# nv-tlabs/LION

Measured on AMD Instinct MI355X. Metric: shapes/sec @1000-step DDIM, Bx2048pts, higher is better.
Workload: dtype f32 (operands of the 3x3x3 voxel convolutions and of the long 1x1 convolutions cut into fp16 hi/lo pairs on the 16-bi...

## Files before the change

lion_amd/csrc/devoxelize.hip:

```cpp
#include "common.h"

namespace {

struct Corners {
  int ix[8];
  float w[8];
};

__device__ __forceinline__ Corners corners_of(float x, float y, float z, int r, int r2) {
  Corners k;
  const float xl = floorf(x), yl = floorf(y), zl = floorf(z);
  const float xd1 = sub_rn(x, xl), yd1 = sub_rn(y, yl), zd1 = sub_rn(z, zl);
  const float xd0 = sub_rn(1.0f, xd1), yd0 = sub_rn(1.0f, yd1), zd0 = sub_rn(1.0f, zd1);
  k.w[0] = mul_rn(mul_rn(xd0, yd0), zd0);
  k.w[1] = mul_rn(mul_rn(xd0, yd0), zd1);
  k.w[2] = mul_rn(mul_rn(xd0, yd1), zd0);
  k.w[3] = mul_rn(mul_rn(xd0, yd1), zd1);
  k.w[4] = mul_rn(mul_rn(xd1, yd0), zd0);
  k.w[5] = mul_rn(mul_rn(xd1, yd0), zd1);
  k.w[6] = mul_rn(mul_rn(xd1, yd1), zd0);
  k.w[7] = mul_rn(mul_rn(xd1, yd1), zd1);
  const int xlo = (int)xl, ylo = (int)yl, zlo = (int)zl;
  const int xs = (xd1 > 0.0f) ? r2 : 0;
  const int ys = (yd1 > 0.0f) ? r : 0;
  const int zs = (zd1 > 0.0f) ? 1 : 0;
  k.ix[0] = xlo * r2 + ylo * r + zlo;
  k.ix[1] = k.ix[0] + zs;
  k.ix[2] = k.ix[0] + ys;
  k.ix[3] = k.ix[2] + zs;
  k.ix[4] = k.ix[0] + xs;
  k.ix[5] = k.ix[4] + zs;
  k.ix[6] = k.ix[4] + ys;
  k.ix[7] = k.ix[6] + zs;
  return k;
}

template <int CT, bool AFF>
__global__ __launch_bounds__(256) void devox_fwd_kernel(const float *__restrict__ coords,
                                                        const float *__restrict__ feat, int C,
                                                        int N, int r, int training,
                                                        float *__restrict__ out,
                                                        int32_t *__restrict__ inds,
                                                        float *__restrict__ wgts,
                                                        const float *__restrict__ scale,
                                                        const float *__restrict__ shift) {
  const int b = blockIdx.z, i = blockIdx.x * blockDim.x + threadIdx.x;
  if (i >= N) return;
  const int r2 = r * r, r3 = r2 * r;
  const float *co = coords + (size_t)b * 3 * N;
  Corners k = corners_of(co[i], co[i + N], co[i + 2 * N], r, r2);
  if (training && blockIdx.y == 0) {
#pragma unroll
    for (int q = 0; q < 8; ++q) {
      wgts[((size_t)b * 8 + q) * N + i] = k.w[q];
      inds[((size_t)b * 8 + q) * N + i] = k.ix[q];
    }
  }
#pragma unroll
  for (int q = 0; q < 8; ++q) k.ix[q] = min(max(k.ix[q], 0), r3 - 1);
  const int c0 = blockIdx.y * CT, c1 = min(C, c0 + CT);
  const float *f = feat + ((size_t)b * C + c0) * r3;
  float *o = out + ((size_t)b * C + c0) * N + i;
  float wsum = 0.f;
  if (AFF) {
    wsum = k.w[0];
#pragma unroll
    for (int q = 1; q < 8; ++q) wsum += k.w[q];
  }
#pragma unroll 4
  for (int c = c0; c < c1; ++c, f += r3, o += N) {
    float v[8];
#pragma unroll
    for (int q = 0; q < 8; ++q) v[q] = f[k.ix[q]];
    float acc = mul_rn(k.w[0], v[0]);
#pragma unroll
    for (int q = 1; q < 8; ++q) acc = add_rn(acc, mul_rn(k.w[q], v[q]));
    if (AFF) acc = acc * scale[(size_t)b * C + c] + shift[(size_t)b * C + c] * wsum;
    *o = acc;
  }
}


template <int LD, bool AFF, bool SPLIT>
__global__ __launch_bounds__(256) void devox_slab_kernel(
    const float *__restrict__ coords, const float *__restrict__ feat, int C, int N, int r, int PX,
    int XS, int CT, int CI, int slab_floats, int training, float *__restrict__ out,
    int32_t *__restrict__ inds, float *__restrict__ wgts, const float *__restrict__ scale,
    const float *__restrict__ shift) {
  extern __shared__ __attribute__((aligned(16))) unsigned char smem[];
  float *lds = reinterpret_cast<float *>(smem);
  constexpr int PP = 8;
  const int tid = threadIdx.x, b = blockIdx.y, c0 = blockIdx.x * CT;
  const int nch = min(CT, C - c0);
  const int r2 = r * r, r3 = r2 * r;
  const float *co = coords + (size_t)b * 3 * N;
  uint16_t *sorted = reinterpret_cast<uint16_t *>(lds + 2 * slab_floats);
  int *scnt = reinterpret_cast<int *>(sorted + ((N + 1) & ~1));
  unsigned *need = reinterpret_cast<unsigned *>(scnt + XS);

  const int ngrp = (nch + CI - 1) / CI;
  const int nit = ngrp * XS;
  auto slab_count4 = [&](int g, int xs) {
    return XS == 1 ? (min(CI, nch - g * CI) * r3) >> 2 : ((min(r, xs * PX + PX + 1) - xs * PX) * r2) >> 2;
  };
  typedef __attribute__((address_space(3))) float lds_float;
  const uint32_t lds_base = (uint32_t)(uintptr_t)(lds_float *)lds;
  const int wave = __builtin_amdgcn_readfirstlane(tid >> 6);
  auto issue = [&](int it) {
    const int g = it / XS, xs = it - g * XS;
    const float4 *src = reinterpret_cast<const float4 *>(feat + ((size_t)b * C + c0 + g * CI) * r3 + (size_t)xs * PX * r2);
    const int n4 = slab_count4(g, xs);
    const uint32_t dst0 = lds_base + (uint32_t)((it & 1) * slab_floats * 4 + wave * 1024);
    const int row0 = XS == 1 ? 0 : xs * PX * r;
#pragma unroll
    for (int j = 0; j < LD; ++j) {
      const int f = tid + j * 256;
      const float4 *gp = src + f;
      const uint32_t dst = __builtin_amdgcn_readfirstlane(dst0 + j * 4096);
      int row = (4 * f) / r;
      if (XS == 1) row %= r2;
      else row += row0;
      bool want = f < n4 && ((need[row >> 5] >> (row & 31)) & 1u);
      if (SPLIT && !want && f < n4) {
        int rowh = (4 * f + 3) / r;
        if (XS == 1) rowh %= r2;
        else rowh += row0;
        want = (need[rowh >> 5] >> (rowh & 31)) & 1u;
      }
      if (want) {
        unsigned keep;
        asm volatile("s_mov_b32 %0, m0\n\ts_mov_b32 m0, %2\n\ts_nop 0\n\tglobal_load_lds_dwordx4 %1, off\n\ts_mov_b32 m0, %0"
                     : "=&s"(keep) : "v"(gp), "s"(dst) : "memory");
      }
    }
  };
  const int nwords = (r2 + 31) >> 5;
  for (int w = tid; w < nwords; w += 256) need[w] = 0u;
  __syncthreads();
  for (int i = tid; i < N; i += 256) {
    const float x = co[i], y = co[i + N];
    const float xl = floorf(x), yl = floorf(y);
    if (xl >= 0.f && yl >= 0.f && xl < (float)r && yl < (float)r) {
      const int x0 = (int)xl, y0 = (int)yl;
      const int x1 = min(x0 + (sub_rn(x, xl) > 0.0f ? 1 : 0), r - 1), y1 = min(y0 + (sub_rn(y, yl) > 0.0f ? 1 : 0), r - 1);
      const int ra = x0 * r + y0, rb = x0 * r + y1, rc = x1 * r + y0, rd = x1 * r + y1;
      atomicOr(&need[ra >> 5], 1u << (ra & 31));
      atomicOr(&need[rb >> 5], 1u << (rb & 31));
      atomicOr(&need[rc >> 5], 1u << (rc & 31));
      atomicOr(&need[rd >> 5], 1u << (rd & 31));
    }
  }
  __syncthreads();
  issue(0);

  for (int s2 = tid; s2 < XS; s2 += 256) scnt[s2] = 0;
  __syncthreads();
  int sl0[PP];
#pragma unroll
  for (int p = 0; p < PP; ++p) {
    const int i = tid + p * 256;
    sl0[p] = -1;
    if (i < N) {
      sl0[p] = min(max((int)floorf(co[i]) / PX, 0), XS - 1);
      if (XS > 1) atomicAdd(&scnt[sl0[p]], 1);
    }
  }
  __syncthreads();
  if (tid == 0) {
    int run = 0;
    for (int s2 = 0; s2 < XS; ++s2) { const int c = scnt[s2]; scnt[s2] = run; run += c; }
  }
  __syncthreads();
#pragma unroll
  for (int p = 0; p < PP; ++p) {
    const int i = tid + p * 256;
    if (i < N) sorted[XS > 1 ? atomicAdd(&scnt[sl0[p]], 1) : i] = (uint16_t)i;
  }
  __syncthreads();

  int ix0[PP], xsl[PP], pid[PP];
  float xd1[PP], yd1[PP], zd1[PP];
#pragma unroll
  for (int p = 0; p < PP; ++p) {
    const int k = tid + p * 256;
    xsl[p] = -1;
    ix0[p] = 0;
    pid[p] = 0;
    xd1[p] = yd1[p] = zd1[p] = 0.f;
    if (k < N) {
      const int i = sorted[k];
      pid[p] = i;
      const float x = co[i], y = co[i + N], z = co[i + 2 * N];
      const Corners kk = corners_of(x, y, z, r, r2);
      if (training && blockIdx.x == 0) {
#pragma unroll
        for (int q = 0; q < 8; ++q) {
          wgts[((size_t)b * 8 + q) * N + i] = kk.w[q];
          inds[((size_t)b * 8 + q) * N + i] = kk.ix[q];
        }
      }
      const float xl = floorf(x), yl = floorf(y), zl = floorf(z);
      xd1[p] = sub_rn(x, xl);
      yd1[p] = sub_rn(y, yl);
      zd1[p] = sub_rn(z, zl);
      ix0[p] = kk.ix[0];
      xsl[p] = min(max((int)xl / PX, 0), XS - 1);
      const int xin = (int)xl - xsl[p] * PX;
      const bool ok = xl >= 0.f && yl >= 0.f && zl >= 0.f && xl < (float)r && yl < (float)r && zl < (float)r &&
                      kk.ix[7] < r3 && xin >= 0 && xin < PX;
      if (!ok) xsl[p] = -2;
    }
  }

  for (int it = 0; it < nit; ++it) {
    const int g = it / XS, xs = it - g * XS;
    const int cg = c0 + g * CI, cin = min(CI, nch - g * CI);
    float *buf = lds + (it & 1) * slab_floats;
    asm volatile("s_waitcnt vmcnt(0)" ::: "memory");
    __syncthreads();
    if (it + 1 < nit) issue(it + 1);
    const int base = xs * PX * r2;
    float *o = out + ((size_t)b * C + cg) * N;
#pragma unroll
    for (int p = 0; p < PP; ++p) {
      if (xsl[p] == xs) {
        const float xd0 = sub_rn(1.0f, xd1[p]), yd0 = sub_rn(1.0f, yd1[p]), zd0 = sub_rn(1.0f, zd1[p]);
        const int xo = (xd1[p] > 0.0f) ? r2 : 0, yo = (yd1[p] > 0.0f) ? r : 0, zo = (zd1[p] > 0.0f) ? 1 : 0;
        const float w0 = mul_rn(mul_rn(xd0, yd0), zd0), w1 = mul_rn(mul_rn(xd0, yd0), zd1[p]);
        const float w2 = mul_rn(mul_rn(xd0, yd1[p]), zd0), w3 = mul_rn(mul_rn(xd0, yd1[p]), zd1[p]);
        const float w4 = mul_rn(mul_rn(xd1[p], yd0), zd0), w5 = mul_rn(mul_rn(xd1[p], yd0), zd1[p]);
        const float w6 = mul_rn(mul_rn(xd1[p], yd1[p]), zd0), w7 = mul_rn(mul_rn(xd1[p], yd1[p]), zd1[p]);
        float wsum = w0;
        if (AFF) { wsum += w1; wsum += w2; wsum += w3; wsum += w4; wsum += w5; wsum += w6; wsum += w7; }
        const float *f0 = buf + (ix0[p] - base);
        for (int ci = 0; ci < cin; ++ci, f0 += r3) {
          const float *f1 = f0 + xo;
          const float v0 = f0[0], v1 = f0[zo], v2 = f0[yo], v3 = f0[yo + zo];
          const float v4 = f1[0], v5 = f1[zo], v6 = f1[yo], v7 = f1[yo + zo];
          float a = mul_rn(w0, v0);
          a = add_rn(a, mul_rn(w1, v1));
          a = add_rn(a, mul_rn(w2, v2));
          a = add_rn(a, mul_rn(w3, v3));
          a = add_rn(a, mul_rn(w4, v4));
          a = add_rn(a, mul_rn(w5, v5));
          a = add_rn(a, mul_rn(w6, v6));
          a = add_rn(a, mul_rn(w7, v7));
          if (AFF) a = a * scale[(size_t)b * C + cg + ci] + shift[(size_t)b * C + cg + ci] * wsum;
          o[(size_t)ci * N + pid[p]] = a;
        }
      } else if (xsl[p] == -2 && xs == 0) {
        for (int ci = 0; ci < cin; ++ci) o[(size_t)ci * N + pid[p]] = 0.f;
      }
    }
  }
}

constexpr int DVR_R = 32, DVR_NT = 512, DVR_PP = 2048 / DVR_NT;
constexpr int DVR_RING_BYTES = 144 * 1024;
constexpr int DVR_NJ = 9;

__device__ __forceinline__ void wait_vm_uniform(int n) {
  n = __builtin_amdgcn_readfirstlane(n);
#define LION_WVM(k) case k: asm volatile("s_waitcnt vmcnt(" #k ")" ::: "memory"); break;
  switch (n < 0 ? 0 : n) {
    LION_WVM(0) LION_WVM(1) LION_WVM(2) LION_WVM(3) LION_WVM(4) LION_WVM(5) LION_WVM(6) LION_WVM(7) LION_WVM(8) LION_WVM(9)
    LION_WVM(10) LION_WVM(11) LION_WVM(12) LION_WVM(13) LION_WVM(14) LION_WVM(15) LION_WVM(16) LION_WVM(17) LION_WVM(18)
    LION_WVM(19) LION_WVM(20) LION_WVM(21) LION_WVM(22) LION_WVM(23) LION_WVM(24) LION_WVM(25) LION_WVM(26) LION_WVM(27)
    LION_WVM(28) LION_WVM(29) LION_WVM(30) LION_WVM(31) LION_WVM(32) LION_WVM(33) LION_WVM(34) LION_WVM(35) LION_WVM(36)
    LION_WVM(37) LION_WVM(38) LION_WVM(39)
  default: asm volatile("s_waitcnt vmcnt(40)" ::: "memory"); break;
  }
#undef LION_WVM
}

template <int G> constexpr int devox_plan_stride() { return 16 + (DVR_NJ * DVR_NT / (G / 4)) * 2 + 2048 * 16 + 2048; }
// ... 298 lines not shown
  }
  __syncthreads();
  const float *g = gy + row * N;
  const int32_t *id = inds + (size_t)b * 8 * N;
  const float *wg = wgts + (size_t)b * 8 * N;
  for (int i = tid; i < N; i += nt) {
    const float gv = a * g[i];
#pragma unroll
    for (int k = 0; k < 8; ++k) {
      const int ix = min(max(id[(size_t)k * N + i], 0), r3 - 1) - lo;
      if (ix >= 0 && ix < part) atomicAdd(slab + ix, mul_rn(wg[(size_t)k * N + i], gv));
    }
  }
  __syncthreads();
  float *o = dx + row * r3 + lo;
  for (int v = tid * 4; v < part; v += nt * 4)
    *reinterpret_cast<float4 *>(o + v) = *reinterpret_cast<const float4 *>(slab + v);
}

__global__ void devox_bwd_atomic_kernel(const float *__restrict__ gy,
                                        const int32_t *__restrict__ inds,
                                        const float *__restrict__ wgts, int C, int N, int r3,
                                        int CT, float *__restrict__ gx) {
  const int b = blockIdx.z, i = blockIdx.x * blockDim.x + threadIdx.x;
  if (i >= N) return;
  int ix[8];
  float w[8];
  for (int q = 0; q < 8; ++q) {
    ix[q] = min(max(inds[((size_t)b * 8 + q) * N + i], 0), r3 - 1);
    w[q] = wgts[((size_t)b * 8 + q) * N + i];
  }
  const int c0 = blockIdx.y * CT, c1 = min(C, c0 + CT);
  for (int c = c0; c < c1; ++c) {
    const float gv = gy[((size_t)b * C + c) * N + i];
    for (int q = 0; q < 8; ++q) atomicAdd(gx + ((size_t)b * C + c) * r3 + ix[q], mul_rn(w[q], gv));
  }
}

}

constexpr int DVR_G = 8;
constexpr size_t DVR_LDS = (size_t)DVR_RING_BYTES + (size_t)2 * (DVR_R * DVR_R * (DVR_R / DVR_G) / 32) * 4 +
                           (size_t)(DVR_NJ * DVR_NT / (DVR_G / 4)) * 2 + 32 * 4 + 16;
static int devox_ring_depth() {
  static const int d = getenv("LION_DEVOX_RING") ? atoi(getenv("LION_DEVOX_RING")) : 4;
  return d < 2 ? 2 : d;
}

template <int MODE>
static int devox_ring_launch(const float *coords, const float *feat, int B, int C, int N, int training, float *out,
                             int32_t *inds, float *wgts, const float *scale, const float *shift, unsigned char *plan,
                             hipStream_t st) {
  int CT = 8;
  while (CT > 1 && (long)B * lion_cdiv(C, CT) < 256) CT >>= 1;
  return lion_with_flags(scale != nullptr, [&](auto AFFINE) {
    return lion_launch<devox_ring_kernel<decltype(AFFINE)::value, DVR_G, MODE>>(
        dim3(lion_cdiv(C, CT), B), DVR_NT, DVR_LDS, st, coords, feat, C, N, CT, training, out, inds, wgts, scale, shift,
        devox_ring_depth(), plan);
  });
}

extern "C" {

static int devox_launch(const float *coords, const float *feat, int B, int C, int N, int r,
                        int training, float *out, int32_t *inds, float *wgts, const float *scale,
                        const float *shift, hipStream_t st) {
  const int r2 = r * r;
  if (r == DVR_R && N <= 2048 && (((uintptr_t)feat) & 15) == 0) {
    return devox_ring_launch<0>(coords, feat, B, C, N, training, out, inds, wgts, scale, shift, nullptr, st);
  }
  if ((r2 % 4) == 0 && N <= 2048 && r2 <= 4608 && (((uintptr_t)feat) & 15) == 0) {
    const int planes_max = 9216 / r2;
    const int PX = planes_max >= r ? r : planes_max - 1;
    const int XS = lion_cdiv(r, PX);
    const int CI = XS == 1 ? (9216 / (r2 * r) < 16 ? 9216 / (r2 * r) : 16) : 1;
    const int ld0 = lion_cdiv((XS == 1 ? CI * r2 * r : (PX + 1) * r2) / 4, 256);
    const int ld = ld0 <= 1 ? 1 : ld0 <= 2 ? 2 : ld0 <= 4 ? 4 : 9;
    const int slab_floats = ld * 1024;
    const size_t lds = (size_t)2 * slab_floats * 4 + (size_t)((N + 1) & ~1) * 2 + (size_t)XS * 4 +
                       (size_t)((r2 + 31) / 32) * 4;
    int CT = 4 * CI;
    while (CT > CI && (long)B * lion_cdiv(C, CT) < 512) CT >>= 1;
    dim3 grid(lion_cdiv(C, CT), B);
    auto slab = [&](auto LD) {
      return lion_with_flags(scale != nullptr, (r & 3) != 0, [&](auto AFFINE, auto SPLIT) {
        return lion_launch<devox_slab_kernel<decltype(LD)::value, decltype(AFFINE)::value, decltype(SPLIT)::value>>(
            grid, 256, lds, st, coords, feat, C, N, r, PX, XS, CT, CI, slab_floats, training, out, inds, wgts, scale, shift);
      });
    };
    return ld <= 1 ? slab(IntC<1>{}) : ld <= 2 ? slab(IntC<2>{}) : ld <= 4 ? slab(IntC<4>{}) : slab(IntC<9>{});
  }
  const int pt = lion_cdiv(N, 256);
  int ct = 16;
  while (ct > 2 && (long)B * pt * lion_cdiv(C, ct) < 2048) ct >>= 1;
  dim3 grid(pt, lion_cdiv(C, ct), B);
  auto fwd = [&](auto CT) {
    return lion_with_flags(scale != nullptr, [&](auto AFFINE) {
      return lion_launch<devox_fwd_kernel<decltype(CT)::value, decltype(AFFINE)::value>>(
          grid, 256, 0, st, coords, feat, C, N, r, training, out, inds, wgts, scale, shift);
    });
  };
  switch (ct) {
  case 16: return fwd(IntC<16>{});
  case 8:  return fwd(IntC<8>{});
  case 4:  return fwd(IntC<4>{});
  default: return fwd(IntC<2>{});
  }
}

int lion_trilinear_devoxelize_forward(const float *coords, const float *feat, int B, int C, int N,
                                      int r, int training, float *out, int32_t *inds, float *wgts,
                                      lionStream_t stream) {
  if (!coords || !feat || !out || B <= 0 || C <= 0 || N <= 0 || r <= 0) return LION_EINVAL;
  if (training && (!inds || !wgts)) return LION_EINVAL;
  return devox_launch(coords, feat, B, C, N, r, training, out, inds, wgts, nullptr, nullptr,
                      static_cast<hipStream_t>(stream));
}

int lion_trilinear_devoxelize_affine_forward(const float *coords, const float *feat, const float *scale,
                                             const float *shift, int B, int C, int N, int r, float *out,
                                             lionStream_t stream) {
  if (!coords || !feat || !out || !scale || !shift || B <= 0 || C <= 0 || N <= 0 || r <= 0) return LION_EINVAL;
  return devox_launch(coords, feat, B, C, N, r, 0, out, nullptr, nullptr, scale, shift,
                      static_cast<hipStream_t>(stream));
}

size_t lion_devoxelize_plan_bytes(int B, int N, int r) {
  if (B <= 0 || N <= 0 || N > 2048 || r != DVR_R) return 0;
  return (size_t)B * devox_plan_stride<DVR_G>();
}

int lion_trilinear_devoxelize_plan(const float *coords, int B, int N, int r, void *plan, size_t plan_bytes,
                                   lionStream_t stream) {
  if (!coords || !plan || B <= 0 || N <= 0) return LION_EINVAL;
  const size_t need = lion_devoxelize_plan_bytes(B, N, r);
  if (!need || (((uintptr_t)plan) & 15) != 0) return LION_EUNSUPPORTED;
  if (plan_bytes < need) return LION_EWORKSPACE;
  return lion_launch<devox_ring_kernel<false, DVR_G, 2>>(dim3(1, B), DVR_NT, DVR_LDS, static_cast<hipStream_t>(stream),
                                                         coords, nullptr, 1, N, 1, 0, nullptr, nullptr, nullptr,
                                                         nullptr, nullptr, devox_ring_depth(),
                                                         static_cast<unsigned char *>(plan));
}

int lion_trilinear_devoxelize_planned_forward(const void *plan, size_t plan_bytes, const float *coords, const float *feat,
                                              const float *scale, const float *shift, int B, int C, int N, int r,
                                              float *out, lionStream_t stream) {
  if (!plan || !coords || !feat || !out || B <= 0 || C <= 0 || N <= 0) return LION_EINVAL;
  if ((scale == nullptr) != (shift == nullptr)) return LION_EINVAL;
  const size_t need = lion_devoxelize_plan_bytes(B, N, r);
  if (!need || (((uintptr_t)plan) & 15) != 0 || (((uintptr_t)feat) & 15) != 0) return LION_EUNSUPPORTED;
  if (plan_bytes < need) return LION_EWORKSPACE;
  hipStream_t st = static_cast<hipStream_t>(stream);
  unsigned char *pl = const_cast<unsigned char *>(static_cast<const unsigned char *>(plan));
  return devox_ring_launch<1>(coords, feat, B, C, N, 0, out, nullptr, nullptr, scale, shift, pl, st);
}

int lion_trilinear_devoxelize_backward(const float *gy, const int32_t *inds, const float *wgts,
                                       int B, int C, int N, int r3, float *gx,
                                       lionStream_t stream) {
  if (!gy || !inds || !wgts || !gx || B <= 0 || C <= 0 || N <= 0 || r3 <= 0) return LION_EINVAL;
  hipStream_t st = static_cast<hipStream_t>(stream);
  if ((size_t)r3 * 4 <= 128 * 1024 && (r3 % 4) == 0) {
    int parts = (size_t)r3 * 4 > 64 * 1024 ? 2 : 1;
    if (r3 % (4 * parts) != 0) parts = 1;
    const size_t lds = (size_t)(r3 / parts) * 4;
    const int nt = r3 >= 16384 ? 1024 : 256;
    return lion_launch<devox_bwd_lds_kernel>(dim3(C, B, parts), nt, lds, st, gy, inds, wgts, C, N, r3, gx);
  }
  hipError_t e = hipMemsetAsync(gx, 0, (size_t)B * C * r3 * 4, st);
  if (e != hipSuccess) return (int)e;
  const int CT = 8;
  return lion_launch<devox_bwd_atomic_kernel>(dim3(lion_cdiv(N, 256), lion_cdiv(C, CT), B), 256, 0, st, gy, inds, wgts,
                                              C, N, r3, CT, gx);
// ... 17 lines not shown
```

lion_amd/csrc/voxelize.hip:

```cpp
#include "common.h"

namespace {

constexpr int VT = 1024;
constexpr int MAXP = 8;
constexpr int LDS_LIMIT = 160 * 1024;
constexpr int PREFETCH_PAD = 2 * 16 * 4;

__device__ __forceinline__ int padv(int v) { return v + (v >> 5); }
__host__ __device__ inline int align4i(int x) { return (x + 3) & ~3; }

__device__ __forceinline__ int lds_slot_add_aggregated(int32_t *arr, int idx, bool valid, int lane) {
  int ret = 0;
  unsigned long long todo = __ballot(valid);
  int singles = 0;
#pragma unroll 1
  for (int it = 0; it < 8 && todo != 0ull && singles < 2; ++it) {
    const int leader = __ffsll((long long)todo) - 1;
    const int k = __shfl(idx, leader, 64);
    const unsigned long long m = __ballot(valid && idx == k) & todo;
    const bool mine = (m >> lane) & 1ull;
    int base = 0;
    if (lane == leader) base = atomicAdd(&arr[k], (int)__popcll(m));
    base = __shfl(base, leader, 64);
// ... 254 lines not shown
  int32_t *uvl_g = plan ? pl.uvl + ((size_t)b * S + slab) * n_words : nullptr;

  const int VPT = (SV + VT - 1) / VT;
  const int v0 = min(tid * VPT, SV), v1 = min(v0 + VPT, SV);
  int lp = 0, lq = 0;
  for (int v = v0; v < v1; ++v) { const int c = (int)hist[padv(v)]; lp += c; lq += (c > 0); }
  const int packed = (lp << 16) | lq;
  const int incl = wave_incl_scan(packed, lane);
  if (lane == 63) iscr[wave] = incl;
  __syncthreads();
  int excl = incl - packed, total = 0;
  for (int w = 0; w < VT / 64; ++w) { const int t = iscr[w]; if (w < wave) excl += t; total += t; }
  const int my_pts = total >> 16, my_occ = total & 0xffff;
  {
    int run = excl >> 16, urun = excl & 0xffff;
    for (int v = v0; v < v1; ++v) {
      const uint32_t c = hist[padv(v)];
      if (c) {
        hist[padv(v)] = ((uint32_t)urun << 16) | c;
        ust[urun] = (run << 16) | (int)c;
        if (uvl_g) uvl_g[urun] = v;
        ++urun;
        run += (int)c;
      }
    }
  }
  __syncthreads();
#pragma unroll
  for (int p = 0; p < NP; ++p) {
    const int i = tid + p * VT;
    const bool in_slab = i < N && myv[p] >= 0 && myv[p] < SV;
    const int a = lds_slot_add_aggregated(slot, in_slab ? padv(myv[p]) : 0, in_slab, lane);
    if (in_slab) tmp[(ust[hist[padv(myv[p])] >> 16] >> 16) + a] = i;
  }
  __syncthreads();
  int posv[NP];
  float invp[NP];
#pragma unroll
  for (int p = 0; p < NP; ++p) {
    const int i = tid + p * VT;
    posv[p] = -1;
    invp[p] = 0.f;
    if (i < N && myv[p] >= 0 && myv[p] < SV) {
      const int h = ust[hist[padv(myv[p])] >> 16];
      const int s = h >> 16, c = h & 0xffff;
      int rank = 0, q = 0;
      for (; q + 8 <= c; q += 8) {
        int t[8];
#pragma unroll
        for (int j = 0; j < 8; ++j) t[j] = tmp[s + q + j];
#pragma unroll
        for (int j = 0; j < 8; ++j) rank += (t[j] < i) ? 1 : 0;
      }
      for (; q < c; ++q) rank += (tmp[s + q] < i) ? 1 : 0;
      posv[p] = s + rank;
      invp[p] = div_rn(1.0f, (float)c);
    }
  }
  if (plan) {
    if (tid == 0) {
      int32_t *h = pl.hdr + ((size_t)b * S + slab) * 4;
      h[0] = my_pts; h[1] = my_occ; h[2] = 0; h[3] = 0;
    }
    int32_t *ust_g = pl.ust + ((size_t)b * S + slab) * n_words;
    for (int u = tid; u < my_occ; u += VT) ust_g[u] = ust[u];
#pragma unroll
    for (int p = 0; p < NP; ++p) {
      const int i = tid + p * VT;
      if (i < N && posv[p] >= 0) {
        pl.pos[(size_t)b * N + i] = (slab << 16) | posv[p];
        pl.inv[(size_t)b * N + i] = invp[p];
      }
    }
    if (feat == nullptr) return;
  }
  for (int v = tid; v < SV; v += VT) {
    const uint32_t h = hist[padv(v)];
    slot[v] = (h & 0xffff) ? (int)(h >> 16) : -1;
  }
  vox_means_and_store<NP>(feat, out, b, C, N, r3, lo, SV, cs, CS, my_pts, my_occ, posv, invp, slot, ust, arena,
                          arena_words, ch_cap);
}

template <int NP, bool READ>
__global__ __launch_bounds__(VT) void vox_scatter_kernel(
    const float *__restrict__ feat, const void *__restrict__ plan, int B, int C, int N, int r3, int S, int CS, int SV,
    int n_words, int arena_words, int ch_cap, float *__restrict__ out, const int32_t *__restrict__ occ_flags, int r, int TD,
    int TH) {
  extern __shared__ __attribute__((aligned(16))) unsigned char smem[];
  int32_t *slot = reinterpret_cast<int32_t *>(smem);
  int32_t *ust = slot + SV;
  int32_t *hdr_s = ust + n_words;
  float *arena = reinterpret_cast<float *>(hdr_s + 64);
  const int tid = threadIdx.x;
  const int W = S * CS;
  const int L = blockIdx.x, grp = L / (8 * W), j8 = L - grp * 8 * W;
  const int b = grp * 8 + (j8 & 7), wq = j8 >> 3, slab = wq % S, cs = wq / S;
  if (b >= B) return;
  const VoxPlanPtrs pl = vox_plan_ptrs(const_cast<void *>(plan), B, N, S);
  const int c_per = (C + CS - 1) / CS, cg_lo = cs * c_per, cg_hi = min(C, cg_lo + c_per);
  if (cg_lo >= cg_hi) return;
  int l_pts = 0, l_occ = 0, l_chm = 1, l_nc = 0;
  {
    const int ls = tid & 63;
    if (ls < S) {
      const int32_t *hs = pl.hdr + ((size_t)b * S + ls) * 4;
      l_pts = hs[0];
      l_occ = hs[1];
      l_chm = min(ch_cap, l_pts > 0 ? min(C, arena_words / ((l_pts | 1) + l_occ)) : C);
      l_nc = l_pts > 0 ? (cg_hi - cg_lo + l_chm - 1) / l_chm : 1;
    }
  }
  int posw[NP];
  float invw[NP];
#pragma unroll
  for (int p = 0; p < NP; ++p) {
    const int i = min(tid + p * VT, N - 1);
    posw[p] = (tid + p * VT < N) ? pl.pos[(size_t)b * N + i] : -1;
    invw[p] = pl.inv[(size_t)b * N + i];
  }
  const unsigned long long empt = __ballot((tid & 63) < S && l_pts == 0);
  int rem = l_nc, ld2 = (((empt >> (tid & 63)) & 1) != 0) ? 1 : 0x7fffff, taken = 0;
  unsigned long long adopted = 0;
  int n_adopted = 0;
#ifndef LION_VOXS_ADOPT
#define LION_VOXS_ADOPT 1
#endif
  if (LION_VOXS_ADOPT && NP >= 2 && empt != 0) {
    for (int it = 0; it < 5 * 16; ++it) {
      int km = (rem << 8) | (63 - (tid & 63)), ka = (ld2 << 8) | (tid & 63);
#pragma unroll
      for (int m = 1; m < 16; m <<= 1) {
        km = max(km, __shfl_xor(km, m));
        ka = min(ka, __shfl_xor(ka, m));
      }
      km = __builtin_amdgcn_readfirstlane(km);
      ka = __builtin_amdgcn_readfirstlane(ka);
      const int smax = 63 - (km & 0xff), nmax = km >> 8, a_ = ka & 0xff, la = ka >> 8;
      if (nmax < 2 || nmax > 256 || la + 2 >= 2 * nmax) break;
      if ((tid & 63) == smax) --rem;
      if ((tid & 63) == a_) {
        ld2 += 2;
        if (++taken == 5) ld2 = 0x7fffff;
      }
      if (a_ == slab) adopted |= (unsigned long long)((smax << 8) | (nmax - 1)) << (12 * n_adopted++);
    }
  }
  if (tid < S) *reinterpret_cast<int4 *>(hdr_s + 4 * tid) = make_int4(l_pts, l_occ, l_chm, rem);
  __syncthreads();
  const int own_nc = __builtin_amdgcn_readfirstlane(hdr_s[4 * slab + 3]);
  n_adopted = __builtin_amdgcn_readfirstlane(n_adopted);
  for (int t = 0; t <= n_adopted; ++t) {
  const int slab_u = __builtin_amdgcn_readfirstlane(t < n_adopted ? (int)((adopted >> (12 * t + 8)) & 0xf) : slab);
  const int k_u = __builtin_amdgcn_readfirstlane(t < n_adopted ? (int)((adopted >> (12 * t)) & 0xff) : 0);
  const int my_pts = __builtin_amdgcn_readfirstlane(hdr_s[4 * slab_u]), my_occ = __builtin_amdgcn_readfirstlane(hdr_s[4 * slab_u + 1]),
            chm_u = __builtin_amdgcn_readfirstlane(hdr_s[4 * slab_u + 2]);
  const int c_begin = cg_lo + k_u * chm_u,
            c_end = t < n_adopted ? min(cg_hi, c_begin + chm_u) : my_pts > 0 ? min(cg_hi, cg_lo + own_nc * chm_u) : cg_hi;
  if (t > 0) __syncthreads();
  int posv[NP];
  float invp[NP];
#pragma unroll
  for (int p = 0; p < NP; ++p) {
    const bool mine = (posw[p] >> 16) == slab_u;
    posv[p] = mine ? (posw[p] & 0xffff) : -1;
    invp[p] = mine ? invw[p] : 0.f;
  }
  if constexpr (READ) {
    __shared__ unsigned char rowneed[1024];
    const int nth = r / TH, ntiles = (r / TD) * nth, row0 = (slab_u * SV) / r, nrows = SV / r;
    const int32_t *fl = occ_flags + (size_t)b * ntiles;
    for (int q = tid; q < nrows; q += VT) {
      const int d = (row0 + q) / r, h = (row0 + q) % r;
      int need = 0;
      for (int dd = max(d - 1, 0); dd <= min(d + 1, r - 1); ++dd)
        for (int hh = max(h - 1, 0); hh <= min(h + 1, r - 1); ++hh) need |= fl[(dd / TD) * nth + hh / TH] & 0xf;
      rowneed[q] = need != 0;
    }
    __syncthreads();
    for (int v = tid; v < SV; v += VT) slot[v] = rowneed[v / r] ? -1 : -2;
  } else {
    for (int v = tid; v < SV; v += VT) slot[v] = -1;
  }
  __syncthreads();
  const int32_t *ust_g = pl.ust + ((size_t)b * S + slab_u) * n_words;
  const int32_t *uvl_g = pl.uvl + ((size_t)b * S + slab_u) * n_words;
  for (int u = tid; u < my_occ; u += VT) {
    ust[u] = ust_g[u];
    slot[uvl_g[u]] = u;
  }
  vox_means_and_store<NP, READ>(feat, out, b, C, N, r3, slab_u * SV, SV, cs, CS, my_pts, my_occ, posv, invp, slot, ust, arena,
                                arena_words, ch_cap, c_begin, c_end);
  }
}

__global__ void vox_index_atomic_kernel(const int32_t *__restrict__ coords, int N, int r,
                                        int32_t *__restrict__ ind, int32_t *__restrict__ cnt) {
  const int b = blockIdx.y, i = blockIdx.x * blockDim.x + threadIdx.x;
  if (i >= N) return;
  const int r2 = r * r, r3 = r2 * r;
  const int32_t *co = coords + (size_t)b * 3 * N;
  const int v = co[i] * r2 + co[i + N] * r + co[i + 2 * N];
  ind[(size_t)b * N + i] = v;
  atomicAdd(cnt + (size_t)b * r3 + min(max(v, 0), r3 - 1), 1);
}

__global__ void vox_scatter_atomic_kernel(const float *__restrict__ feat,
                                          const int32_t *__restrict__ ind,
                                          const int32_t *__restrict__ cnt, int C, int N, int r3,
                                          int CT, float *__restrict__ out) {
  const int b = blockIdx.z, i = blockIdx.x * blockDim.x + threadIdx.x;
  if (i >= N) return;
  const int pos = min(max(ind[(size_t)b * N + i], 0), r3 - 1);
  const int cur = cnt[(size_t)b * r3 + pos];
  if (cur <= 0) return;
  const float inv = div_rn(1.0f, (float)cur);
  const int c0 = blockIdx.y * CT, c1 = min(C, c0 + CT);
  for (int c = c0; c < c1; ++c)
    atomicAdd(out + ((size_t)b * C + c) * r3 + pos, mul_rn(feat[((size_t)b * C + c) * N + i], inv));
}

__global__ __launch_bounds__(VT) void p1_kernel(const float *__restrict__ coords, int N, int r,
                                                int normalize, float eps,
                                                float *__restrict__ norm_coords,
                                                int32_t *__restrict__ vox) {
  __shared__ float fscr[64];
  const int tid = threadIdx.x, lane = tid & 63, wave = tid >> 6, b = blockIdx.x;
  const float *co = coords + (size_t)b * 3 * N;
  float mean[3];
  for (int a = 0; a < 3; ++a) {
    float part = 0.f;
    for (int k = tid; k < N; k += VT) part = add_rn(part, co[k + (size_t)a * N]);
    for (int s = 1; s < 64; s <<= 1) part = add_rn(part, __shfl_xor(part, s, 64));
    __syncthreads();
    if (lane == 0) fscr[wave] = part;
    __syncthreads();
    float v = fscr[lane & 15];
    for (int s = 1; s < 16; s <<= 1) v = add_rn(v, __shfl_xor(v, s, 64));
    mean[a] = div_rn(v, (float)N);
  }
  float denom = 1.0f;
  if (normalize) {
    float mx = 0.f;
    for (int k = tid; k < N; k += VT) {
      const float x = sub_rn(co[k], mean[0]), y = sub_rn(co[k + N], mean[1]),
                  z = sub_rn(co[k + 2 * (size_t)N], mean[2]);
      const float nr = sqrt_rn(add_rn(add_rn(mul_rn(x, x), mul_rn(y, y)), mul_rn(z, z)));
      mx = nr > mx ? nr : mx;
    }
    for (int s = 1; s < 64; s <<= 1) { const float o = __shfl_xor(mx, s, 64); mx = o > mx ? o : mx; }
    __syncthreads();
    if (lane == 0) fscr[wave] = mx;
    __syncthreads();
    float m2 = fscr[lane & 15];
    for (int s = 1; s < 16; s <<= 1) { const float o = __shfl_xor(m2, s, 64); m2 = o > m2 ? o : m2; }
    denom = add_rn(mul_rn(m2, 2.0f), eps);
  }
  const float rf = (float)r, hi = (float)(r - 1);
  for (int a = 0; a < 3; ++a)
    for (int k = tid; k < N; k += VT) {
      float v = sub_rn(co[k + (size_t)a * N], mean[a]);
// ... 119 lines not shown
                                                       ind, cnt, C, N, r3, CT, out))
      return e;
  }
  return 0;
}

}

extern "C" {

int lion_abi_version(void) { return 1; }

size_t lion_avg_voxelize_workspace_bytes(int B, int C, int N, int r) {
  (void)C;
  if (B <= 0 || N <= 0 || r <= 0) return 0;
  return make_plan(B, C, N, r).total;
}

int lion_avg_voxelize_forward(const float *feat, const int32_t *coords, int B, int C, int N, int r,
                              float *out, int32_t *ind, int32_t *cnt, void *ws, size_t ws_bytes,
                              lionStream_t stream) {
  if (!feat || !coords) return LION_EINVAL;
  return voxelize_impl(feat, coords, nullptr, B, C, N, r, 0, 0.f, out, nullptr, ind, cnt, ws,
                       ws_bytes, static_cast<hipStream_t>(stream));
}

int lion_voxelize_points_forward(const float *feat, const float *coords, int B, int C, int N,
                                 int r, int normalize, float eps, float *out, float *norm_coords,
                                 int32_t *ind, int32_t *cnt, void *ws, size_t ws_bytes,
                                 lionStream_t stream) {
  if (!coords) return LION_EINVAL;
  return voxelize_impl(feat, nullptr, coords, B, C, N, r, normalize, eps, out, norm_coords, ind,
                       cnt, ws, ws_bytes, static_cast<hipStream_t>(stream));
}

size_t lion_voxel_plan_bytes(int B, int N, int r) {
  if (B <= 0 || N <= 0 || r <= 0 || (long)r * r * r > (1L << 30)) return 0;
  const VoxPlan p = make_plan(B, 0, N, r);
  if (!p.fast) return 0;
  return vox_plan_words(B, N, p.S) * 4;
}

int lion_voxel_index(const float *coords, int B, int N, int r, int normalize, float eps, float *norm_coords,
                     int32_t *ind, int32_t *cnt, void *plan, size_t plan_bytes, lionStream_t stream) {
  if (!coords || !plan || !norm_coords) return LION_EINVAL;
  const size_t need = lion_voxel_plan_bytes(B, N, r);
  if (need == 0) return LION_EUNSUPPORTED;
  if (plan_bytes < need) return LION_EWORKSPACE;
  return voxelize_impl(nullptr, nullptr, coords, B, 0, N, r, normalize, eps, nullptr, norm_coords, ind, cnt, nullptr, 0,
                       static_cast<hipStream_t>(stream), plan);
}

static int voxel_scatter_impl(const float *feat, const void *plan, size_t plan_bytes, int B, int C, int N, int r, float *out,
                              const int32_t *occ_flags, lionStream_t stream);

int lion_voxel_scatter(const float *feat, const void *plan, size_t plan_bytes, int B, int C, int N, int r, float *out,
                       lionStream_t stream) {
  return voxel_scatter_impl(feat, plan, plan_bytes, B, C, N, r, out, nullptr, stream);
}

int lion_voxel_scatter_read(const float *feat, const void *plan, size_t plan_bytes, int B, int C, int N, int r,
                            const int32_t *occ_m1, float *out, lionStream_t stream) {
  if (!occ_m1) return LION_EINVAL;
  if (r != 16 && r != 32) return LION_EUNSUPPORTED;
  return voxel_scatter_impl(feat, plan, plan_bytes, B, C, N, r, out, occ_m1, stream);
}

static int voxel_scatter_impl(const float *feat, const void *plan, size_t plan_bytes, int B, int C, int N, int r, float *out,
                              const int32_t *occ_flags, lionStream_t stream) {
  if (!feat || !plan || !out || B <= 0 || C <= 0 || N <= 0 || r <= 0) return LION_EINVAL;
  const size_t need = lion_voxel_plan_bytes(B, N, r);
  if (need == 0 || (((uintptr_t)out) & 15) != 0) return LION_EUNSUPPORTED;
  if (plan_bytes < need) return LION_EWORKSPACE;
  const VoxPlan p0 = make_plan(B, C, N, r);
  if (!p0.fast) return LION_EUNSUPPORTED;
  VoxPlan p = p0;
#ifndef LION_VOXS_TWO
#define LION_VOXS_TWO 0
#endif
  const bool two_per_cu = LION_VOXS_TWO || N <= VT;
  if (two_per_cu) {
    int CS = 1;
    while ((long)B * p.S * CS < 512 && C / (CS * 2) >= 8) CS *= 2;
    p.CS = CS;
  }
  const size_t lds_limit = (two_per_cu ? (size_t)LDS_LIMIT / 2 : (size_t)LDS_LIMIT) - PREFETCH_PAD - (occ_flags ? 1024 + 64 : 0);
  const size_t fixed = ((size_t)p.SV + (size_t)p.n_words + 64) * 4;
  const size_t nocc = (size_t)(N < p.SV ? N : p.SV);
  const size_t want = ((size_t)N + 1 + nocc) * C * 4;
  const size_t avail = fixed < lds_limit ? lds_limit - fixed : 0;
  const size_t arena = want < avail ? want : avail;
  if (arena / 4 < (size_t)N + 1 + nocc) return LION_EUNSUPPORTED;
  const size_t lds = fixed + arena + PREFETCH_PAD;
  const int grid = ((B + 7) / 8) * 8 * p.S * p.CS;
  const int r3 = r * r * r;
  hipStream_t st = static_cast<hipStream_t>(stream);
  int occ_td = 0, occ_th = 0;
  if (occ_flags)
    if (int e = lion_internal_sparse_tile_dims(r, &occ_td, &occ_th)) return e;
  return lion_with_flags(occ_flags != nullptr, [&](auto READ) {
    return vox_np_dispatch(p.NP, [&](auto NPV) {
      return lion_launch<vox_scatter_kernel<decltype(NPV)::value, decltype(READ)::value>>(
          grid, VT, lds, st, feat, plan, B, C, N, r3, p.S, p.CS, p.SV, p.n_words, (int)(arena / 4), 64, out, occ_flags, r,
          occ_td, occ_th);
    });
  });
}

int lion_avg_voxelize_backward(const float *gy, const int32_t *ind, const int32_t *cnt, int B,
                               int C, int N, int r3, float *gx, lionStream_t stream) {
  if (!gy || !ind || !cnt || !gx || B <= 0 || C <= 0 || N <= 0 || r3 <= 0) return LION_EINVAL;
  const int CT = 8;
  return lion_launch<vox_grad_kernel>(dim3(lion_cdiv(N, 256), lion_cdiv(C, CT), B), 256, 0,
                                      static_cast<hipStream_t>(stream), gy, ind, cnt, C, N, r3, CT, gx);
}

}
```

Baseline: 5.651.

## Add single-slab devoxelize path and NP==1 voxel-scatter fast path

```diff
diff --git a/lion_amd/csrc/devoxelize.hip b/lion_amd/csrc/devoxelize.hip
--- a/lion_amd/csrc/devoxelize.hip
+++ b/lion_amd/csrc/devoxelize.hip
@@ -81,15 +81,18 @@
 }
 
 
-template <int LD, bool AFF, bool SPLIT>
+template <int LD, bool AFF, bool SPLIT, bool ONE>
 __global__ __launch_bounds__(256) void devox_slab_kernel(
     const float *__restrict__ coords, const float *__restrict__ feat, int C, int N, int r, int PX,
-    int XS, int CT, int CI, int slab_floats, int training, float *__restrict__ out,
+    int XS_rt, int CT, int CI, int slab_floats, int training, float *__restrict__ out,
     int32_t *__restrict__ inds, float *__restrict__ wgts, const float *__restrict__ scale,
     const float *__restrict__ shift) {
+  static_assert(!(ONE && SPLIT), "the single-slab form fetches whole grids: there is no row-end rule to apply");
+  constexpr bool FILT = !ONE;
   extern __shared__ __attribute__((aligned(16))) unsigned char smem[];
   float *lds = reinterpret_cast<float *>(smem);
   constexpr int PP = 8;
+  const int XS = ONE ? 1 : XS_rt;
   const int tid = threadIdx.x, b = blockIdx.y, c0 = blockIdx.x * CT;
   const int nch = min(CT, C - c0);
   const int r2 = r * r, r3 = r2 * r;
@@ -117,15 +120,20 @@
       const int f = tid + j * 256;
       const float4 *gp = src + f;
       const uint32_t dst = __builtin_amdgcn_readfirstlane(dst0 + j * 4096);
-      int row = (4 * f) / r;
-      if (XS == 1) row %= r2;
-      else row += row0;
-      bool want = f < n4 && ((need[row >> 5] >> (row & 31)) & 1u);
-      if (SPLIT && !want && f < n4) {
-        int rowh = (4 * f + 3) / r;
-        if (XS == 1) rowh %= r2;
-        else rowh += row0;
-        want = (need[rowh >> 5] >> (rowh & 31)) & 1u;
+      bool want;
+      if (FILT) {
+        int row = (4 * f) / r;
+        if (XS == 1) row %= r2;
+        else row += row0;
+        want = f < n4 && ((need[row >> 5] >> (row & 31)) & 1u);
+        if (SPLIT && !want && f < n4) {
+          int rowh = (4 * f + 3) / r;
+          if (XS == 1) rowh %= r2;
+          else rowh += row0;
+          want = (need[rowh >> 5] >> (rowh & 31)) & 1u;
+        }
+      } else {
+        want = f < n4;
       }
       if (want) {
         unsigned keep;
@@ -134,49 +142,60 @@
       }
     }
   };
-  const int nwords = (r2 + 31) >> 5;
-  for (int w = tid; w < nwords; w += 256) need[w] = 0u;
-  __syncthreads();
-  for (int i = tid; i < N; i += 256) {
-    const float x = co[i], y = co[i + N];
-    const float xl = floorf(x), yl = floorf(y);
-    if (xl >= 0.f && yl >= 0.f && xl < (float)r && yl < (float)r) {
-      const int x0 = (int)xl, y0 = (int)yl;
-      const int x1 = min(x0 + (sub_rn(x, xl) > 0.0f ? 1 : 0), r - 1), y1 = min(y0 + (sub_rn(y, yl) > 0.0f ? 1 : 0), r - 1);
-      const int ra = x0 * r + y0, rb = x0 * r + y1, rc = x1 * r + y0, rd = x1 * r + y1;
-      atomicOr(&need[ra >> 5], 1u << (ra & 31));
-      atomicOr(&need[rb >> 5], 1u << (rb & 31));
-      atomicOr(&need[rc >> 5], 1u << (rc & 31));
-      atomicOr(&need[rd >> 5], 1u << (rd & 31));
-    }
-  }
-  __syncthreads();
-  issue(0);
-
-  for (int s2 = tid; s2 < XS; s2 += 256) scnt[s2] = 0;
-  __syncthreads();
-  int sl0[PP];
-#pragma unroll
-  for (int p = 0; p < PP; ++p) {
-    const int i = tid + p * 256;
-    sl0[p] = -1;
-    if (i < N) {
-      sl0[p] = min(max((int)floorf(co[i]) / PX, 0), XS - 1);
-      if (XS > 1) atomicAdd(&scnt[sl0[p]], 1);
-    }
-  }
-  __syncthreads();
-  if (tid == 0) {
-    int run = 0;
-    for (int s2 = 0; s2 < XS; ++s2) { const int c = scnt[s2]; scnt[s2] = run; run += c; }
-  }
-  __syncthreads();
-#pragma unroll
-  for (int p = 0; p < PP; ++p) {
-    const int i = tid + p * 256;
-    if (i < N) sorted[XS > 1 ? atomicAdd(&scnt[sl0[p]], 1) : i] = (uint16_t)i;
-  }
-  __syncthreads();
+  float cx[PP], cy[PP], cz[PP];
+  if constexpr (ONE) {
+#pragma unroll
+    for (int p = 0; p < PP; ++p) {
+      const int i = tid + p * 256;
+      cx[p] = cy[p] = cz[p] = 0.f;
+      if (i < N) { cx[p] = co[i]; cy[p] = co[i + N]; cz[p] = co[i + 2 * N]; }
+    }
+    issue(0);
+  } else {
+    const int nwords = (r2 + 31) >> 5;
+    for (int w = tid; w < nwords; w += 256) need[w] = 0u;
+    __syncthreads();
+    for (int i = tid; i < N; i += 256) {
+      const float x = co[i], y = co[i + N];
+      const float xl = floorf(x), yl = floorf(y);
+      if (xl >= 0.f && yl >= 0.f && xl < (float)r && yl < (float)r) {
+        const int x0 = (int)xl, y0 = (int)yl;
+        const int x1 = min(x0 + (sub_rn(x, xl) > 0.0f ? 1 : 0), r - 1), y1 = min(y0 + (sub_rn(y, yl) > 0.0f ? 1 : 0), r - 1);
+        const int ra = x0 * r + y0, rb = x0 * r + y1, rc = x1 * r + y0, rd = x1 * r + y1;
+        atomicOr(&need[ra >> 5], 1u << (ra & 31));
+        atomicOr(&need[rb >> 5], 1u << (rb & 31));
+        atomicOr(&need[rc >> 5], 1u << (rc & 31));
+        atomicOr(&need[rd >> 5], 1u << (rd & 31));
+      }
+    }
+    __syncthreads();
+    issue(0);
+
+    for (int s2 = tid; s2 < XS; s2 += 256) scnt[s2] = 0;
+    __syncthreads();
+    int sl0[PP];
+#pragma unroll
+    for (int p = 0; p < PP; ++p) {
+      const int i = tid + p * 256;
+      sl0[p] = -1;
+      if (i < N) {
+        sl0[p] = min(max((int)floorf(co[i]) / PX, 0), XS - 1);
+        if (XS > 1) atomicAdd(&scnt[sl0[p]], 1);
+      }
+    }
+    __syncthreads();
+    if (tid == 0) {
+      int run = 0;
+      for (int s2 = 0; s2 < XS; ++s2) { const int c = scnt[s2]; scnt[s2] = run; run += c; }
+    }
+    __syncthreads();
+#pragma unroll
+    for (int p = 0; p < PP; ++p) {
+      const int i = tid + p * 256;
+      if (i < N) sorted[XS > 1 ? atomicAdd(&scnt[sl0[p]], 1) : i] = (uint16_t)i;
+    }
+    __syncthreads();
+  }
 
   int ix0[PP], xsl[PP], pid[PP];
   float xd1[PP], yd1[PP], zd1[PP];
@@ -188,9 +207,9 @@
     pid[p] = 0;
     xd1[p] = yd1[p] = zd1[p] = 0.f;
     if (k < N) {
-      const int i = sorted[k];
+      const int i = ONE ? k : (int)sorted[k];
       pid[p] = i;
-      const float x = co[i], y = co[i + N], z = co[i + 2 * N];
+      const float x = ONE ? cx[p] : co[i], y = ONE ? cy[p] : co[i + N], z = ONE ? cz[p] : co[i + 2 * N];
       const Corners kk = corners_of(x, y, z, r, r2);
       if (training && blockIdx.x == 0) {
 #pragma unroll
@@ -655,13 +674,19 @@
     int CT = 4 * CI;
     while (CT > CI && (long)B * lion_cdiv(C, CT) < 512) CT >>= 1;
     dim3 grid(lion_cdiv(C, CT), B);
-    auto slab = [&](auto LD) {
-      return lion_with_flags(scale != nullptr, (r & 3) != 0, [&](auto AFFINE, auto SPLIT) {
-        return lion_launch<devox_slab_kernel<decltype(LD)::value, decltype(AFFINE)::value, decltype(SPLIT)::value>>(
+    auto slab = [&](auto LD, auto SPLIT, auto ONE) {
+      return lion_with_flags(scale != nullptr, [&](auto AFFINE) {
+        return lion_launch<devox_slab_kernel<decltype(LD)::value, decltype(AFFINE)::value, decltype(SPLIT)::value,
+                                             decltype(ONE)::value>>(
             grid, 256, lds, st, coords, feat, C, N, r, PX, XS, CT, CI, slab_floats, training, out, inds, wgts, scale, shift);
       });
     };
-    return ld <= 1 ? slab(IntC<1>{}) : ld <= 2 ? slab(IntC<2>{}) : ld <= 4 ? slab(IntC<4>{}) : slab(IntC<9>{});
+    if (XS > 1) {
+      if (ld != 9) return LION_EUNSUPPORTED;
+      return (r & 3) != 0 ? slab(IntC<9>{}, BoolC<true>{}, BoolC<false>{}) : slab(IntC<9>{}, BoolC<false>{}, BoolC<false>{});
+    }
+    return ld <= 1 ? slab(IntC<1>{}, BoolC<false>{}, BoolC<true>{}) : ld <= 2 ? slab(IntC<2>{}, BoolC<false>{}, BoolC<true>{})
+         : ld <= 4 ? slab(IntC<4>{}, BoolC<false>{}, BoolC<true>{}) : slab(IntC<9>{}, BoolC<false>{}, BoolC<true>{});
   }
   const int pt = lion_cdiv(N, 256);
   int ct = 16;
diff --git a/lion_amd/csrc/voxelize.hip b/lion_amd/csrc/voxelize.hip
--- a/lion_amd/csrc/voxelize.hip
+++ b/lion_amd/csrc/voxelize.hip
@@ -360,6 +360,14 @@
                           arena_words, ch_cap);
 }
 
+__device__ __forceinline__ bool vox_row_has_reader(const int32_t *fl, int row, int r, int TD, int TH, int nth) {
+  const int d = row / r, h = row % r;
+  int need = 0;
+  for (int dd = max(d - 1, 0); dd <= min(d + 1, r - 1); ++dd)
+    for (int hh = max(h - 1, 0); hh <= min(h + 1, r - 1); ++hh) need |= fl[(dd / TD) * nth + hh / TH] & 0xf;
+  return need != 0;
+}
+
 template <int NP, bool READ>
 __global__ __launch_bounds__(VT) void vox_scatter_kernel(
     const float *__restrict__ feat, const void *__restrict__ plan, int B, int C, int N, int r3, int S, int CS, int SV,
@@ -378,6 +386,42 @@
   const VoxPlanPtrs pl = vox_plan_ptrs(const_cast<void *>(plan), B, N, S);
   const int c_per = (C + CS - 1) / CS, cg_lo = cs * c_per, cg_hi = min(C, cg_lo + c_per);
   if (cg_lo >= cg_hi) return;
+  if constexpr (NP == 1) {
+    const int ls = tid & 63;
+    int l_pts = 0, l_occ = 0;
+    if (ls < S) {
+      const int32_t *hs = pl.hdr + ((size_t)b * S + ls) * 4;
+      l_pts = hs[0];
+      l_occ = hs[1];
+    }
+    const int i = min(tid, N - 1);
+    const int posw = tid < N ? pl.pos[(size_t)b * N + i] : -1;
+    const float invw = pl.inv[(size_t)b * N + i];
+    const int uc = min(tid, min(N, SV) - 1);
+    const int u_st = pl.ust[((size_t)b * S + slab) * n_words + uc], u_vl = pl.uvl[((size_t)b * S + slab) * n_words + uc];
+    if constexpr (READ) {
+      const int nth = r / TH, ntiles = (r / TD) * nth, row0 = (slab * SV) / r, nrows = SV / r;
+      const int32_t *fl = occ_flags + (size_t)b * ntiles;
+      for (int q = tid; q < nrows; q += VT) {
+        const int sv = vox_row_has_reader(fl, row0 + q, r, TD, TH, nth) ? -1 : -2;
+        for (int z = 0; z < r; z += 4) *reinterpret_cast<int4 *>(slot + q * r + z) = make_int4(sv, sv, sv, sv);
+      }
+    } else {
+      for (int v = tid; v < SV; v += VT) slot[v] = -1;
+    }
+    asm volatile("s_waitcnt lgkmcnt(0)\n\ts_barrier" ::: "memory");
+    const int my_pts = __builtin_amdgcn_readlane(l_pts, slab), my_occ = __builtin_amdgcn_readlane(l_occ, slab);
+    if (tid < my_occ) {
+      ust[tid] = u_st;
+      slot[u_vl] = tid;
+    }
+    const bool mine = (posw >> 16) == slab;
+    const int posv[1] = {mine ? (posw & 0xffff) : -1};
+    const float invp[1] = {mine ? invw : 0.f};
+    vox_means_and_store<1, READ>(feat, out, b, C, N, r3, slab * SV, SV, cs, CS, my_pts, my_occ, posv, invp, slot, ust, arena,
+                                 arena_words, ch_cap, cg_lo, cg_hi);
+    return;
+  }
   int l_pts = 0, l_occ = 0, l_chm = 1, l_nc = 0;
   {
     const int ls = tid & 63;
@@ -448,13 +492,7 @@
     __shared__ unsigned char rowneed[1024];
     const int nth = r / TH, ntiles = (r / TD) * nth, row0 = (slab_u * SV) / r, nrows = SV / r;
     const int32_t *fl = occ_flags + (size_t)b * ntiles;
-    for (int q = tid; q < nrows; q += VT) {
-      const int d = (row0 + q) / r, h = (row0 + q) % r;
-      int need = 0;
-      for (int dd = max(d - 1, 0); dd <= min(d + 1, r - 1); ++dd)
-        for (int hh = max(h - 1, 0); hh <= min(h + 1, r - 1); ++hh) need |= fl[(dd / TD) * nth + hh / TH] & 0xf;
-      rowneed[q] = need != 0;
-    }
+    for (int q = tid; q < nrows; q += VT) rowneed[q] = vox_row_has_reader(fl, row0 + q, r, TD, TH, nth);
     __syncthreads();
     for (int v = tid; v < SV; v += VT) slot[v] = rowneed[v / r] ? -1 : -2;
   } else {
@@ -740,6 +778,7 @@
   if (two_per_cu) {
     int CS = 1;
     while ((long)B * p.S * CS < 512 && C / (CS * 2) >= 8) CS *= 2;
+    while (CS > 1 && (long)p.SV * ((C + CS - 1) / CS) < 8192 && (long)B * p.S * (CS / 2) >= 256) CS /= 2;
     p.CS = CS;
   }
   const size_t lds_limit = (two_per_cu ? (size_t)LDS_LIMIT / 2 : (size_t)LDS_LIMIT) - PREFETCH_PAD - (occ_flags ? 1024 + 64 : 0);
```

Result: faster. 5.729, median of 6 (+1.4%).
